# xiaojino/RUArt

Measured on AMD Instinct MI355X. Metric: VQA samples/sec fwd+bwd (B=64, q=30, ocr=100), higher is better.
Workload: dtype f16 MFMA + block-scaled fp8 (e4m3) MFMA correction, f32 accumulate / residual stream; 1 GPU; RUArt training step, synthetic ST-VQA-shaped batch: B=64/GPU, q=30 words, 100 OCR items, 36 objects, bert-base 12x768 frozen, SDNet trunk fwd+bwd, Adamax; global_batch=64, real_wordpieces_per_batch=42738, parallelism=dp1, mode=train

## Files before the change

### include/ruart_hip.h

```cpp
#ifndef RUART_HIP_H
#define RUART_HIP_H
#include <stddef.h>

#ifdef __cplusplus
extern "C" {
#endif

#define RUART_DT_F32 0
#define RUART_DT_BF16 1
#define RUART_DT_F16 2
#define RUART_ACT_NONE 0
#define RUART_ACT_GELU 1
#define RUART_ACT_RELU 2

const char* ruart_version(void);

int ruart_gemm_16_nt(const void* A, int lda, const void* W, int ldw, const float* bias, const void* residual, int ldr,
                     int residual_dtype, void* C, int ldc, int out_dtype, int M, int N, int K, int act, int in_dtype,
                     void* stream);
size_t ruart_gemm_16_tail_ws_bytes(int M, int N, int K, int cus);
int ruart_gemm_16_nt_ws(const void* A, int lda, const void* W, int ldw, const float* bias, const void* residual, int ldr, int residual_dtype,
                        void* C, int ldc, int out_dtype, int M, int N, int K, int act, int in_dtype, void* tail_ws, size_t tail_ws_bytes, int cus,
                        void* stream);
int ruart_gemm_16c_nt(const void* A16, const void* A8, int lda, const void* W16, const void* W8, int ldw, const float* bias,
// ... 138 lines not shown
size_t ruart_bert_workspace_bytes(const ruart_bert_model* m, int n_rows);
int ruart_bert_set_correction(int qkv, int ao, int ff1, int ff2, unsigned long long layer_mask);
int ruart_bert_forward(const ruart_bert_model* m, const ruart_bert_batch* b, void* layers_out, void* workspace,
                       size_t workspace_bytes, void* stream);

size_t ruart_bert_workspace_bytes_folded(const ruart_bert_model* m, int n_rows);
int ruart_bert_forward_folded(const ruart_bert_model* m, const ruart_bert_batch* b, void* layers_pre, float* ln_stats, void* workspace,
                              size_t workspace_bytes, void* stream);
int ruart_gemm_16c_nt_fold(const void* A16, const void* A8, int lda, const void* W16, const void* W8, int ldw, const float* bias, int kind,
                           const float* in_part, int in_np, const float* colc, float wscale, const float* residual, int ldr,
                           const float* res_part, int res_np, const float* res_gamma, const float* res_beta, void* C, int ldc, void* C16,
                           void* C8, float* out_part, int M, int N, int K, int stat_len, float eps, void* stream);
int ruart_gemm_16_nt_fold(const void* A, int lda, const void* W, int ldw, const float* bias, int kind, const float* in_part, int in_np,
                          const float* colc, float wscale, const void* residual, int ldr, const float* res_part, int res_np,
                          const float* res_gamma, const float* res_beta, void* C, int ldc, float* out_part, int M, int N, int K, int stat_len,
                          float eps, int dtype, void* stream);
int ruart_rows_stats_finish(const float* part, int np, int rows, float inv_h, float eps, float* stats, void* stream);
int ruart_bert_pool_mix_ln(const float* layers_pre, long long layer_stride, int ldl, int n_layers, const float* ln_stats,
                           long long stats_stride, const float* ln_gamma, const float* ln_beta, const int* span_start,
                           const int* span_start_last, const int* span_len, const int* dst_row, const float* layer_w, float* out, int ldo,
                           int n_words, int H, void* stream);
int ruart_bert_pool_ln_set_variant(int reg_tables);
int ruart_bert_pool_mix_ln_bwd(const float* layers_pre, long long layer_stride, int ldl, int n_layers, const float* ln_stats,
                               long long stats_stride, const float* ln_gamma, const float* ln_beta, const int* span_start,
                               const int* span_start_last, const int* span_len, const int* dst_row, const float* grad_out, int ldg,
                               float* partial_ws, float* grad_layer_w, int n_words, int H, void* stream);

int ruart_attn_fwd(const float* pa, const float* pk, const float* v, const unsigned char* mask, const float* diag, int diag_len,
                   int relu, float* out, float* probs, int B, int L1, int L2, int h, int D3, void* stream);
int ruart_attn_bwd(const float* pa, const float* pk, const float* v, const float* probs, const float* grad_out, const float* diag,
                   int diag_len, int relu, float* grad_pa, float* grad_pk, float* grad_v, float* grad_diag_partial,
                   float* ds_ws , int B, int L1, int L2, int h, int D3, void* stream);
int ruart_attn_set_prefetch(int on);
int ruart_attn_fwd_pscale(const float* pa, const float* pk, const float* v, const unsigned char* mask, const float* diag, int diag_len,
                          int relu, const float* prob_scale, float* out, float* probs, int B, int L1, int L2, int h, int D3,
                          void* stream);
int ruart_attn_bwd_pscale(const float* pa, const float* pk, const float* v, const float* probs, const float* grad_out, const float* diag,
                          int diag_len, int relu, const float* prob_scale, float* grad_pa, float* grad_pk, float* grad_v,
                          float* grad_diag_partial, float* ds_ws, int B, int L1, int L2, int h, int D3, void* stream);

int ruart_whole_ln_fwd(const float* x, float* y, float* stats, float* ws, long long n, float eps, void* stream);
int ruart_whole_ln_bwd(const float* y, const float* grad_y, const float* stats, float* grad_x, float* ws, long long n,
                       void* stream);

int ruart_whole_ln_blocks(void);
int ruart_whole_ln_partials(const float* x, const float* x2, float* part, long long n, void* stream);
int ruart_whole_ln_var_global(const float* x, long long n, const float* part_all, int world, long long n_total, float* part2,
                              void* stream);
int ruart_whole_ln_apply_global(const float* x, float* y, long long n, float eps, const float* part_all, const float* part2_all,
                                int world, long long n_total, float* stats, void* stream);
int ruart_whole_ln_bwd_global(const float* y, const float* grad_y, const float* stats, float* grad_x, long long n,
                              const float* part_all, int world, long long n_total, void* stream);

int ruart_scorer_fwd(const float* x, const float* u1, const float* u2, const float* uh, const float* w, const float* bna,
                     const unsigned char* mask, float* probs, float* a_out, int B, int L, int D, int ES, int mask_flag, void* stream);
int ruart_scorer_bwd(const float* x, const float* u1, const float* u2, const float* uh, const float* w, const float* probs,
                     const float* a_in, const float* gprobs, float* gx, float* gu1, float* gu2, float* guh, float* gw_part,
                     float* gb_part, int B, int L, int D, int ES, void* stream);

int ruart_lstm_set_variant(int variant);
int ruart_lstm_fwd(const float* xproj, const float* w_hh, float* y, float* gates, float* cells, float* hprev, int B, int T, int h,
                   int ndir, void* stream);
int ruart_lstm_bwd(const float* grad_y, const float* w_hh, const float* gates, const float* cells, float* grad_xproj, int B,
                   int T, int h, int ndir, void* stream);

int ruart_lstm_pack_params(const float* w_ih, const float* w_ih_r, const float* b_ih, const float* b_hh, const float* b_ih_r,
// ... 56 lines not shown
```

### ruart_amd/csrc/sdnet_attention.hip

```cpp
#include <cstdlib>
#include "common.h"
#include "ruart_hip.h"

#define CH 64
#define LDA_ 66
#define LDB_ 80
#define NTW 6
#define ATTN_MAX_L2 384

int* ruart_nan_flag_ptr = nullptr;

__device__ __forceinline__ f32x4_t mma16(const float* As, int lda, const float* Bs, int sbk, int sbj, int Kc, f32x4_t acc) {
  const int lane = threadIdx.x & 63, r = lane & 15, q = lane >> 4;
  for (int kk = 0; kk < Kc; kk += 4) acc = __builtin_amdgcn_mfma_f32_16x16x4f32(As[r * lda + kk + q], Bs[(kk + q) * sbk + r * sbj], acc, 0, 0, 0);
  return acc;
}

struct Act {
  int relu;
  const float* diag;
  int diag_len;
  __device__ __forceinline__ float operator()(float v, int col) const {
    if (relu) v = fmaxf(v, 0.f);
    if (diag_len == 1) v *= diag[0];
// ... 574 lines not shown
    const int kc = min(CH, (L1 - r0 + 3) & ~3);
    o = mma16(xt_s, LDA_, y_s + wave * 16, LDB_, 1, kc, o);
    if (ri == nr - 1) {
      const int n = n0 + wave * 16 + (lane & 15);
#pragma unroll
      for (int r = 0; r < 4; ++r) {
        const int j = j0 + (lane >> 4) * 4 + r;
        if (j < L2 && n < N) {
          const size_t at = (size_t)j * N + n;
          C[at] = (out_gate && out_gate[at] <= 0.f) ? 0.f : o[r];
        }
      }
      o = (f32x4_t){0.f, 0.f, 0.f, 0.f};
    }
    ri = rn;
    ni = nx;
  }
}

__global__ __launch_bounds__(256) void attn_bwd_kv_pf_kernel(const float* __restrict__ a, const float* __restrict__ probs,
                                                             const float* __restrict__ dS, const float* __restrict__ gout,
                                                             float* __restrict__ grad_k, float* __restrict__ grad_v, int L1, int L2, int h,
                                                             int D3, const float* __restrict__ pk, int relu,
                                                             const float* __restrict__ diag, int diag_len,
                                                             const float* __restrict__ pscale) {
  const int b = blockIdx.y, j0 = blockIdx.x * 16;
  float* xt_s = dsm;
  float* y_s = xt_s + 16 * LDA_;
  const size_t pb = (size_t)b * L1 * L2;
  tn_product_pf(dS + pb, L1, L2, j0, a + (size_t)b * L1 * h, h, grad_k + (size_t)b * L2 * h, xt_s, y_s, Act{relu, diag, diag_len},
                (relu && pk) ? pk + (size_t)b * L2 * h : nullptr, nullptr);
  tn_product_pf(probs + pb, L1, L2, j0, gout + (size_t)b * L1 * D3, D3, grad_v + (size_t)b * L2 * D3, xt_s, y_s, no_act(), nullptr,
                pscale ? pscale + pb : nullptr);
}

#define WLN_BLOCKS 256
__device__ __forceinline__ float grid_partial_total(const float* part, float* red) {
  float s = (threadIdx.x < WLN_BLOCKS) ? part[threadIdx.x] : 0.f;
  return block_sum<4>(s, red);
}

#define WLN_FOR4(n4, ...)                                                                          \
  for (long long i_ = blockIdx.x * 256LL + threadIdx.x; i_ < (n4); i_ += 4LL * 256 * WLN_BLOCKS) { \
    long long ix_[4];                                                                              \
    bool ok_[4];                                                                                   \
    _Pragma("unroll") for (int u_ = 0; u_ < 4; ++u_) {                                             \
      const long long j_ = i_ + (long long)u_ * 256 * WLN_BLOCKS;                                  \
      ok_[u_] = j_ < (n4);                                                                         \
      ix_[u_] = ok_[u_] ? j_ : (n4) - 1;                                                           \
    }                                                                                              \
    __VA_ARGS__                                                                                    \
  }
__device__ __forceinline__ bool wln_vec_ok(const void* a, const void* b, const void* c, long long n) {
  return ((n & 3) == 0) && (((reinterpret_cast<uintptr_t>(a) | reinterpret_cast<uintptr_t>(b) | reinterpret_cast<uintptr_t>(c)) & 15) == 0) && n >= 4;
}

__global__ __launch_bounds__(256) void wln_sum_kernel(const float* __restrict__ x, const float* __restrict__ x2, long long n,
                                                      float* __restrict__ part) {
  __shared__ float red[4];
  float s = 0.f, t = 0.f;
  if (wln_vec_ok(x, x2, nullptr, n)) {
    const f32x4_t* x4 = reinterpret_cast<const f32x4_t*>(x);
    const f32x4_t* y4 = reinterpret_cast<const f32x4_t*>(x2);
    const long long n4 = n >> 2;
    if (x2) {
      WLN_FOR4(n4, f32x4_t a[4], b[4];
// ... 148 lines not shown
               y4[ix_[u]] = o;
               bad |= !(o[0] == o[0]) || !(o[1] == o[1]) || !(o[2] == o[2]) || !(o[3] == o[3]);
             })
  } else {
    for (long long i = blockIdx.x * 256LL + threadIdx.x; i < n; i += 256LL * WLN_BLOCKS) {
      const float o = (x[i] - mean) * rstd;
      y[i] = o;
      bad |= !(o == o);
    }
  }
  if (bad && nan_flag) atomicOr(nan_flag, 1);
}
__global__ __launch_bounds__(256) void wln_bwd_global_kernel(const float* __restrict__ y, const float* __restrict__ gy,
                                                             const float* __restrict__ stats, float* __restrict__ gx, long long n,
                                                             const float* __restrict__ part_all, int world, long long n_total) {
  __shared__ float red[4];
  const float mg = wln_ranks_total(part_all, 2 * WLN_BLOCKS, world, red) / (float)n_total;
  const float mgy = wln_ranks_total(part_all + WLN_BLOCKS, 2 * WLN_BLOCKS, world, red) / (float)n_total;
  const float rstd = stats[1];
  if (wln_vec_ok(y, gy, gx, n)) {
    const f32x4_t* y4 = reinterpret_cast<const f32x4_t*>(y);
    const f32x4_t* g4 = reinterpret_cast<const f32x4_t*>(gy);
    f32x4_t* o4 = reinterpret_cast<f32x4_t*>(gx);
    const long long n4 = n >> 2;
    WLN_FOR4(n4, f32x4_t a[4], b[4];
             _Pragma("unroll") for (int u = 0; u < 4; ++u) { a[u] = y4[ix_[u]]; b[u] = g4[ix_[u]]; }
             _Pragma("unroll") for (int u = 0; u < 4; ++u) if (ok_[u]) o4[ix_[u]] = rstd * (b[u] - mg - a[u] * mgy);)
  } else {
    for (long long i = blockIdx.x * 256LL + threadIdx.x; i < n; i += 256LL * WLN_BLOCKS) gx[i] = rstd * (gy[i] - mg - y[i] * mgy);
  }
}

static bool g_attn_prefetch = !(getenv("RUART_ATTN_PREFETCH") && atoi(getenv("RUART_ATTN_PREFETCH")) == 0);
template <typename K> static void attn_big_lds(K kern) { hipFuncSetAttribute((const void*)kern, hipFuncAttributeMaxDynamicSharedMemorySize, 160 * 1024); }
static void attn_allow_big_lds() {
  static bool done = (attn_big_lds(attn_fwd_kernel), attn_big_lds(attn_bwd_q_kernel), attn_big_lds(attn_fwd_pf_kernel<12>),
                      attn_big_lds(attn_fwd_pf_kernel<16>), attn_big_lds(attn_fwd_pf_kernel<28>), attn_big_lds(attn_fwd_pf_kernel<32>),
                      attn_big_lds(attn_bwd_q_pf_kernel<12>), attn_big_lds(attn_bwd_q_pf_kernel<16>), attn_big_lds(attn_bwd_q_pf_kernel<28>),
                      attn_big_lds(attn_bwd_q_pf_kernel<32>), true);
  (void)done;
}

static size_t attn_lds_bytes(int L2) {
  const int L2p = (L2 + 15) & ~15;
  const int ldS = ((L2p + 31) / 32) * 32 + 2;
  return sizeof(float) * (size_t)(16 * LDA_ + 16 * ldS + L2p * LDB_);
}

__global__ __launch_bounds__(256) void attn1_fwd_kernel(const float* __restrict__ a, const float* __restrict__ k,
                                                        const float* __restrict__ v, const unsigned char* __restrict__ mask,
                                                        float* __restrict__ out, float* __restrict__ probs, int L2, int h, int D3,
                                                        int* __restrict__ nan_flag) {
  __shared__ float p_s[ATTN_MAX_L2];
  __shared__ float red[4];
  const int b = blockIdx.x, tid = threadIdx.x, lane = tid & 63, wave = tid >> 6;
  const float* ab = a + (size_t)b * h;
  const float* kb = k + (size_t)b * L2 * h;
  const float* vb = v + (size_t)b * L2 * D3;
  for (int j0 = wave * 4; j0 < L2; j0 += 16) {
    float s[4] = {0.f, 0.f, 0.f, 0.f};
    for (int d = lane; d < h; d += 64) {
      const float av = ab[d];
#pragma unroll
      for (int u = 0; u < 4; ++u)
        if (j0 + u < L2) s[u] = fmaf(av, kb[(size_t)(j0 + u) * h + d], s[u]);
    }
#pragma unroll
    for (int u = 0; u < 4; ++u) {
      const float t = wave_sum(s[u]);
      if (lane == 0 && j0 + u < L2) p_s[j0 + u] = mask[(size_t)b * L2 + j0 + u] ? t : -INFINITY;
    }
  }
  __syncthreads();
  float mx = -INFINITY;
  for (int j = tid; j < L2; j += 256) mx = fmaxf(mx, p_s[j]);
  mx = block_max<4>(mx, red);
  float sum = 0.f;
  for (int j = tid; j < L2; j += 256) {
    const float e = expf(p_s[j] - mx);
// ... 70 lines not shown
#pragma unroll
      for (int u = 0; u < 8; ++u) g = fmaf(ds_s[j + u], t[u], g);
    }
    for (; j < L2; ++j) g = fmaf(ds_s[j], kb[(size_t)j * h + d], g);
    grad_a[(size_t)b * h + d] = g;
  }
  for (int e = tid; e < L2 * h; e += 256) grad_k[(size_t)b * L2 * h + e] = ds_s[e / h] * ab[e % h];
  for (int e = tid; e < L2 * D3; e += 256) grad_v[(size_t)b * L2 * D3 + e] = pb[e / D3] * gb[e % D3];
}

extern "C" int ruart_attn_fwd(const float* a, const float* k, const float* v, const unsigned char* mask, const float* diag,
                              int diag_len, int relu, float* out, float* probs, int B, int L1, int L2, int h, int D3, void* stream) {
  RUART_ENTRY();
  return ruart_attn_fwd_pscale(a, k, v, mask, diag, diag_len, relu, nullptr, out, probs, B, L1, L2, h, D3, stream);
}

extern "C" int ruart_attn_fwd_pscale(const float* a, const float* k, const float* v, const unsigned char* mask, const float* diag,
                                     int diag_len, int relu, const float* prob_scale, float* out, float* probs, int B, int L1, int L2,
                                     int h, int D3, void* stream) {
  RUART_ENTRY();
  if (B <= 0 || L1 <= 0 || L2 <= 0 || L2 > ATTN_MAX_L2 || h <= 0 || D3 <= 0) return (int)hipErrorInvalidValue;
  if (diag_len != 0 && diag_len != 1 && diag_len != h) return (int)hipErrorInvalidValue;
  if (L1 == 1 && !relu && diag_len == 0 && !prob_scale) {
    hipLaunchKernelGGL(attn1_fwd_kernel, dim3(B), dim3(256), 0, (hipStream_t)stream, a, k, v, mask, out, probs, L2, h, D3,
                       ruart_nan_flag_ptr);
    RUART_CHECK_LAUNCH();
    return 0;
  }
  const dim3 grid(ceil_div(L1, 16), B), block(256);
  attn_allow_big_lds();
  const int L2p = (L2 + 15) & ~15;
#define RUART_AF(U) hipLaunchKernelGGL(attn_fwd_pf_kernel<U>, grid, block, attn_lds_bytes(L2), (hipStream_t)stream, a, k, v, mask, out, probs, \
                                       L1, L2, h, D3, ruart_nan_flag_ptr, relu, diag_len ? diag : nullptr, diag_len, prob_scale)
  if (!g_attn_prefetch || L2p > 128)
    hipLaunchKernelGGL(attn_fwd_kernel, grid, block, attn_lds_bytes(L2), (hipStream_t)stream, a, k, v, mask, out, probs, L1, L2, h, D3,
                       ruart_nan_flag_ptr, relu, diag_len ? diag : nullptr, diag_len, prob_scale);
  else if (L2p <= 48) RUART_AF(12);
  else if (L2p <= 64) RUART_AF(16);
  else if (L2p <= 112) RUART_AF(28);
  else RUART_AF(32);
#undef RUART_AF
  RUART_CHECK_LAUNCH();
  return 0;
}

extern "C" int ruart_attn_set_prefetch(int on) {
  RUART_ENTRY();
  g_attn_prefetch = on != 0;
  return 0;
}

extern "C" int ruart_attn_bwd(const float* a, const float* k, const float* v, const float* probs, const float* grad_out,
                              const float* diag, int diag_len, int relu, float* grad_a, float* grad_k, float* grad_v,
                              float* grad_diag, float* ds_ws, int B, int L1, int L2, int h, int D3, void* stream) {
  RUART_ENTRY();
  return ruart_attn_bwd_pscale(a, k, v, probs, grad_out, diag, diag_len, relu, nullptr, grad_a, grad_k, grad_v, grad_diag, ds_ws, B, L1,
                               L2, h, D3, stream);
}

extern "C" int ruart_attn_bwd_pscale(const float* a, const float* k, const float* v, const float* probs, const float* grad_out,
                                     const float* diag, int diag_len, int relu, const float* prob_scale, float* grad_a, float* grad_k,
                                     float* grad_v, float* grad_diag, float* ds_ws, int B, int L1, int L2, int h, int D3,
                                     void* stream) {
  RUART_ENTRY();
  if (B <= 0 || L1 <= 0 || L2 <= 0 || L2 > ATTN_MAX_L2 || h <= 0 || D3 <= 0) return (int)hipErrorInvalidValue;
  if (diag_len != 0 && diag_len != 1 && diag_len != h) return (int)hipErrorInvalidValue;
  if (L1 == 1 && !relu && diag_len == 0 && !prob_scale) {
    hipLaunchKernelGGL(attn1_bwd_kernel, dim3(B), dim3(256), 0, (hipStream_t)stream, a, k, v, probs, grad_out, grad_a, grad_k, grad_v,
                       L2, h, D3);
    RUART_CHECK_LAUNCH();
    return 0;
  }
  const bool act = relu || diag_len;
  const float* dg = diag_len ? diag : nullptr;
  attn_allow_big_lds();
  const int L2p = (L2 + 15) & ~15;
#define RUART_AQ(U) hipLaunchKernelGGL(attn_bwd_q_pf_kernel<U>, dim3(ceil_div(L1, 16), B), dim3(256), attn_lds_bytes(L2), (hipStream_t)stream, \
                                       k, v, probs, grad_out, grad_a, ds_ws, L1, L2, h, D3, act ? a : nullptr, relu, dg, diag_len,           \
                                       (diag_len > 1) ? grad_diag : nullptr, prob_scale)
  if (!g_attn_prefetch || L2p > 128)
    hipLaunchKernelGGL(attn_bwd_q_kernel, dim3(ceil_div(L1, 16), B), dim3(256), attn_lds_bytes(L2), (hipStream_t)stream, k, v, probs,
                       grad_out, grad_a, ds_ws, L1, L2, h, D3, act ? a : nullptr, relu, dg, diag_len,
                       (diag_len > 1) ? grad_diag : nullptr, prob_scale);
  else if (L2p <= 48) RUART_AQ(12);
  else if (L2p <= 64) RUART_AQ(16);
  else if (L2p <= 112) RUART_AQ(28);
  else RUART_AQ(32);
#undef RUART_AQ
  RUART_CHECK_LAUNCH();
  const size_t lds = sizeof(float) * (16 * LDA_ + CH * LDB_);
  if (g_attn_prefetch)
    hipLaunchKernelGGL(attn_bwd_kv_pf_kernel, dim3(ceil_div(L2, 16), B), dim3(256), lds, (hipStream_t)stream, a, probs, ds_ws, grad_out,
                       grad_k, grad_v, L1, L2, h, D3, k, relu, dg, diag_len, prob_scale);
  else
    hipLaunchKernelGGL(attn_bwd_kv_kernel, dim3(ceil_div(L2, 16), B), dim3(256), lds, (hipStream_t)stream, a, probs, ds_ws, grad_out,
                       grad_k, grad_v, L1, L2, h, D3, k, relu, dg, diag_len, prob_scale);
  RUART_CHECK_LAUNCH();
  return 0;
}

extern "C" int ruart_whole_ln_fwd(const float* x, float* y, float* stats, float* ws, long long n, float eps, void* stream) {
  RUART_ENTRY();
  if (n <= 0) return (int)hipErrorInvalidValue;
  hipStream_t s = (hipStream_t)stream;
  hipLaunchKernelGGL(wln_sum_kernel, dim3(WLN_BLOCKS), dim3(256), 0, s, x, (const float*)nullptr, n, ws);
  hipLaunchKernelGGL(wln_var_kernel, dim3(WLN_BLOCKS), dim3(256), 0, s, x, n, ws, ws + 2 * WLN_BLOCKS);
  hipLaunchKernelGGL(wln_apply_kernel, dim3(WLN_BLOCKS), dim3(256), 0, s, x, y, n, eps, ws, ws + 2 * WLN_BLOCKS, stats, ruart_nan_flag_ptr);
  RUART_CHECK_LAUNCH();
  return 0;
}

extern "C" int ruart_whole_ln_bwd(const float* y, const float* grad_y, const float* stats, float* grad_x, float* ws, long long n,
                                  void* stream) {
  RUART_ENTRY();
  if (n <= 0) return (int)hipErrorInvalidValue;
  hipStream_t s = (hipStream_t)stream;
  hipLaunchKernelGGL(wln_sum_kernel, dim3(WLN_BLOCKS), dim3(256), 0, s, grad_y, y, n, ws);
  hipLaunchKernelGGL(wln_bwd_kernel, dim3(WLN_BLOCKS), dim3(256), 0, s, y, grad_y, stats, grad_x, n, ws);
  RUART_CHECK_LAUNCH();
  return 0;
}

extern "C" int ruart_whole_ln_blocks(void) { return WLN_BLOCKS; }

// ... 85 lines not shown
```

### ruart_amd/hip.py

```python
import ctypes
import os
from ctypes import POINTER, Structure, c_char_p, c_double, c_float, c_int, c_longlong, c_size_t, c_uint, c_ulonglong, c_void_p

import torch

_HERE = os.path.dirname(os.path.abspath(__file__))
LIB_PATH = os.path.join(_HERE, "libruart_hip.so")

DT_F32, DT_BF16, DT_F16 = 0, 1, 2
ACT_NONE, ACT_GELU, ACT_RELU = 0, 1, 2
TORCH_DTYPE = {DT_F32: torch.float32, DT_BF16: torch.bfloat16, DT_F16: torch.float16}
PRECISION = {"fp32": DT_F32, "bf16": DT_BF16, "fp16": DT_F16, "x3": DT_F32, "fp16c": DT_F32}


class BertModelC(Structure):
    _fields_ = [("hidden", c_int), ("n_heads", c_int), ("n_layers", c_int), ("intermediate", c_int), ("dtype", c_int),
                ("ln_eps", c_float),
                ("word_emb", c_void_p), ("pos_emb", c_void_p), ("type_emb", c_void_p), ("emb_ln_g", c_void_p), ("emb_ln_b", c_void_p),
                ("w_qkv", POINTER(c_void_p)), ("b_qkv", POINTER(c_void_p)),
                ("w_ao", POINTER(c_void_p)), ("b_ao", POINTER(c_void_p)),
                ("ln1_g", POINTER(c_void_p)), ("ln1_b", POINTER(c_void_p)),
                ("w_ff1", POINTER(c_void_p)), ("b_ff1", POINTER(c_void_p)),
                ("w_ff2", POINTER(c_void_p)), ("b_ff2", POINTER(c_void_p)),
                ("ln2_g", POINTER(c_void_p)), ("ln2_b", POINTER(c_void_p)), ("f32_gemm", c_int), ("corr8", c_int),
# ... 69 lines not shown
    "ruart_weight_prep_batch": (_I, [POINTER(WPrepItemC), _I, _P]),
    "ruart_colsum_bf16": (_I, [_P, _I, _I, _I, _P, _I, _P, _P]),
    "ruart_transpose16": (_I, [_P, _I, _P, _I, _I, _I, _I, _P]),
    "ruart_splitk_reduce": (_I, [_P, _LL, _I, _P, _LL, _F, _I, _P]),
    "ruart_mix_rows": (_I, [_P, _LL, _I, _I, _P, _P, _I, _I, _I, _P]),
    "ruart_mix_rows_bwd": (_I, [_P, _LL, _I, _I, _P, _I, _P, _P, _I, _I, _P]),
    "ruart_rows_ln_to_16": (_I, [_P, _LL, _I, _P, _LL, _P, _P, _P, _LL, _I, _I, _I, _I, _I, _P]),
    "ruart_attn_train_fwd": (_I, [_P, _I, _P, _I, _I, _I, _I, _P, _P, _P, _F, _U, _P]),
    "ruart_attn_train_bwd": (_I, [_P, _I, _P, _I, _P, _I, _I, _I, _I, _P, _P, _P, _F, _U, _P, _P]),
    "ruart_attn_train_fwd_long": (_I, [_P, _I, _P, _I, _I, _I, _I, _P, _P, _P, _P, _F, _U, _P, _P]),
    "ruart_attn_train_bwd_long": (_I, [_P, _I, _P, _I, _P, _I, _I, _I, _I, _P, _P, _P, _P, _P, _F, _U, _P, _P, _P, _P, _P]),
    "ruart_gemm_f32_nt": (_I, [_P, _I, _P, _I, _P, _P, _I, _P, _I, _I, _I, _I, _I, _P]),
    "ruart_bert_embed_ln": (_I, [_P, _P, _P, _P, _P, _P, _P, _F, _P, _I, _I, _I, _I, _P]),
    "ruart_rows_layernorm": (_I, [_P, _I, _P, _P, _F, _P, _I, _I, _I, _I, _P]),
    "ruart_bert_attention": (_I, [_P, _I, _P, _I, _I, _I, _I, _I, _P, _P, _P, _P, _P, _P, _P, _I, _P, _P, _P, _P, _P]),
    "ruart_bert_pool_set_variant": (_I, [_I]),
    "ruart_bert_pool_mix": (_I, [_P, _LL, _I, _I, _I, _P, _P, _P, _P, _P, _P, _I, _I, _I, _P]),
    "ruart_bert_pool_mix_bwd": (_I, [_P, _LL, _I, _I, _I, _P, _P, _P, _P, _P, _I, _P, _P, _I, _I, _P]),
    "ruart_rows_gather": (_I, [_P, _I, _P, _LL, _P, _LL, _I, _P, _LL, _P, _LL, _I, _P, _LL, _P, _LL, _I, _P]),
    "ruart_cast_f32_to_16": (_I, [_P, _P, _I, _LL, _F, _P]),
    "ruart_bert_workspace_bytes": (_SZ, [POINTER(BertModelC), _I]),
    "ruart_bert_forward": (_I, [POINTER(BertModelC), POINTER(BertBatchC), _P, _P, _SZ, _P]),
    "ruart_bert_workspace_bytes_folded": (_SZ, [POINTER(BertModelC), _I]),
    "ruart_bert_forward_folded": (_I, [POINTER(BertModelC), POINTER(BertBatchC), _P, _P, _P, _SZ, _P]),
    "ruart_gemm_16c_nt_fold": (_I, [_P, _P, _I, _P, _P, _I, _P, _I, _P, _I, _P, _F, _P, _I, _P, _I, _P, _P, _P, _I, _P, _P, _P, _I, _I, _I, _I, _F, _P]),
    "ruart_gemm_16_nt_fold": (_I, [_P, _I, _P, _I, _P, _I, _P, _I, _P, _F, _P, _I, _P, _I, _P, _P, _P, _I, _P, _I, _I, _I, _I, _F, _I, _P]),
    "ruart_rows_stats_finish": (_I, [_P, _I, _I, _F, _F, _P, _P]),
    "ruart_bert_pool_mix_ln": (_I, [_P, _LL, _I, _I, _P, _LL, _P, _P, _P, _P, _P, _P, _P, _P, _I, _I, _I, _P]),
    "ruart_bert_pool_ln_set_variant": (_I, [_I]),
    "ruart_bert_pool_mix_ln_bwd": (_I, [_P, _LL, _I, _I, _P, _LL, _P, _P, _P, _P, _P, _P, _P, _I, _P, _P, _I, _I, _P]),
    "ruart_attn_fwd": (_I, [_P, _P, _P, _P, _P, _I, _I, _P, _P, _I, _I, _I, _I, _I, _P]),
    "ruart_attn_bwd": (_I, [_P, _P, _P, _P, _P, _P, _I, _I, _P, _P, _P, _P, _P, _I, _I, _I, _I, _I, _P]),
    "ruart_attn_set_prefetch": (_I, [_I]),
    "ruart_attn_fwd_pscale": (_I, [_P, _P, _P, _P, _P, _I, _I, _P, _P, _P, _I, _I, _I, _I, _I, _P]),
    "ruart_attn_bwd_pscale": (_I, [_P, _P, _P, _P, _P, _P, _I, _I, _P, _P, _P, _P, _P, _P, _I, _I, _I, _I, _I, _P]),
    "ruart_whole_ln_fwd": (_I, [_P, _P, _P, _P, _LL, _F, _P]),
    "ruart_whole_ln_bwd": (_I, [_P, _P, _P, _P, _P, _LL, _P]),
    "ruart_whole_ln_blocks": (_I, []),
    "ruart_whole_ln_partials": (_I, [_P, _P, _P, _LL, _P]),
    "ruart_whole_ln_var_global": (_I, [_P, _LL, _P, _I, _LL, _P, _P]),
    "ruart_whole_ln_apply_global": (_I, [_P, _P, _LL, _F, _P, _P, _I, _LL, _P, _P]),
    "ruart_whole_ln_bwd_global": (_I, [_P, _P, _P, _P, _LL, _P, _I, _LL, _P]),
    "ruart_scorer_fwd": (_I, [_P, _P, _P, _P, _P, _P, _P, _P, _P, _I, _I, _I, _I, _I, _P]),
    "ruart_scorer_bwd": (_I, [_P, _P, _P, _P, _P, _P, _P, _P, _P, _P, _P, _P, _P, _P, _I, _I, _I, _I, _P]),
    "ruart_lstm_set_variant": (_I, [_I]),
    "ruart_lstm_pack_params": (_I, [_P, _P, _P, _P, _P, _P, _P, _P, _P, _P, _P, _I, _I, _I, _P]),
    "ruart_lstm_fwd": (_I, [_P, _P, _P, _P, _P, _P, _I, _I, _I, _I, _P]),
    "ruart_lstm_bwd": (_I, [_P, _P, _P, _P, _P, _I, _I, _I, _I, _P]),
    "ruart_rows_scale": (_I, [_P, _I, _P, _I, _P, _P, _I, _I, _I, _P]),
    "ruart_lstm_cell_fwd": (_I, [_P, _P, _P, _P, _P, _P, _I, _I, _I, _P]),
    "ruart_lstm_cell_bwd": (_I, [_P, _P, _P, _P, _P, _P, _P, _P, _I, _I, _I, _P]),
    "ruart_set_nan_flag": (_I, [_P]),
    "ruart_grad_norm_clip": (_I, [_P, _P, _P, _P, _I, _F, _P, _P, _P, _P]),
    "ruart_adamax_step": (_I, [_P, _P, _P, _P, _P, _P, _P, _I, _P, _P, _F, _F, _F, _P]),
    "ruart_embedding_bwd_sorted": (_I, [_P, _P, _P, _P, _I, _I, _P, _P]),
    "ruart_embedding_bwd_split": (_I, [_P, _P, _P, _I, _P, _P, _I, _I, _P, _P, _P]),
    "ruart_phoc_table": (_I, [_P, _P, _I, _P, _I, _P, _P]),
    "ruart_gemm_bf16_tn": (_I, [_P, _LL, _P, _LL, _P, _I, _I, _I, _I, _P, _SZ, _P]),
    "ruart_gemm_x3_tn_grouped_ws": (_SZ, [POINTER(X3TnProblemC), _I]),
    "ruart_gemm_x3_tn_grouped": (_I, [POINTER(X3TnProblemC), _I, _P, _SZ, _P]),
    "ruart_gemm_x3_plan": (_I, [_I, _I, _I, _I, _I, POINTER(c_int), POINTER(_SZ)]),
    "ruart_gemm_x3": (_I, [_P, _LL, _LL, _P, _LL, _LL, _P, _P, _I, _I, _P, _I, _I,
                           _I, _I, _P, _SZ, _P, _P, _F, _P, _I, _P]),
    "ruart_gemm_x1": (_I, [_P, _LL, _LL, _P, _LL, _LL, _P, _P, _I, _I, _P, _I, _I,
                           _I, _I, _P, _SZ, _P, _P, _F, _P, _I, _P]),
    "ruart_stream_create_cu_masked": (_I, [_I, POINTER(c_void_p)]),
# ... 150 lines not shown
```

Before: 2870 samples/s.

## Add LDS-resident attention kernels that stage whole K/V panels per block

Adds resident-panel variants of the SDNet attention forward, backward-dQ and backward-dK/dV kernels for L2 up to 128. These stage entire key/value (or dS/probs) panels into up to 160 KiB of LDS once, using bulk register-buffered loads, and reuse them across several 16-row query tiles per block. The goal is to cut repeated global reloads and per-tile staging overhead. The forward and dQ paths only run when RUART_ATTN_RESIDENT is positive. The dK/dV path runs by default unless that variable is negative, so it replaces the prefetch kernel and changes grid shape and occupancy.

```diff
diff --git a/include/ruart_hip.h b/include/ruart_hip.h
--- a/include/ruart_hip.h
+++ b/include/ruart_hip.h
@@ -194,6 +194,8 @@
                    int diag_len, int relu, float* grad_pa, float* grad_pk, float* grad_v, float* grad_diag_partial,
                    float* ds_ws , int B, int L1, int L2, int h, int D3, void* stream);
 int ruart_attn_set_prefetch(int on);
+int ruart_attn_set_resident(int tiles);
+int ruart_attn_get_resident(int* tiles);
 int ruart_attn_fwd_pscale(const float* pa, const float* pk, const float* v, const unsigned char* mask, const float* diag, int diag_len,
                           int relu, const float* prob_scale, float* out, float* probs, int B, int L1, int L2, int h, int D3,
                           void* stream);
diff --git a/ruart_amd/csrc/sdnet_attention.hip b/ruart_amd/csrc/sdnet_attention.hip
--- a/ruart_amd/csrc/sdnet_attention.hip
+++ b/ruart_amd/csrc/sdnet_attention.hip
@@ -630,6 +630,403 @@
                 (relu && pk) ? pk + (size_t)b * L2 * h : nullptr, nullptr);
   tn_product_pf(probs + pb, L1, L2, j0, gout + (size_t)b * L1 * D3, D3, grad_v + (size_t)b * L2 * D3, xt_s, y_s, no_act(), nullptr,
                 pscale ? pscale + pb : nullptr);
+}
+
+#define RES_U 32
+#define RES_NT 2
+#define RES_LDS_MAX (160 * 1024)
+
+__host__ __device__ __forceinline__ int res_lda(int n) { return ((n + 31) / 32) * 32 + 2; }
+__host__ __device__ __forceinline__ int res_ldb(int n) { const int m = (n + 15) & ~15; return (m & 31) ? m : m + 16; }
+
+struct RPanel {
+  const float* src;
+  int ld, r0, rows, c0, cols, nr_pad, nc_pad;
+};
+__device__ __forceinline__ int rp_quads(const RPanel& p) { return ((p.nr_pad + 15) >> 4) * ((p.nc_pad + 63) >> 6); }
+
+__device__ __forceinline__ float res_ldg(const float* __restrict__ base, unsigned byte_off) {
+  return *reinterpret_cast<const float*>(reinterpret_cast<const char*>(base) + byte_off);
+}
+
+template <int U, int MUL>
+struct Bulk {
+  float v[U];
+  float m[MUL == 2 ? U : (MUL == 1 ? U / 4 : 1)];
+  __device__ __forceinline__ void load(const RPanel& p, int q0, const float* __restrict__ mul = nullptr) {
+    const int lane = threadIdx.x & 63, w = __builtin_amdgcn_readfirstlane(threadIdx.x >> 6);
+    const int NRQ = (p.nr_pad + 15) >> 4;
+    const float* msrc = mul ? mul : p.src;
+    int ci = q0 / NRQ, rq = q0 - ci * NRQ;
+#pragma unroll
+    for (int qq = 0; qq < U / 4; ++qq) {
+      {
+        const unsigned cc = 4u * (unsigned)min(p.c0 + ci * 64 + lane, p.cols - 1);
+        if (MUL == 1) m[qq] = mul ? res_ldg(msrc, cc) : 1.f;
+#pragma unroll
+        for (int j = 0; j < 4; ++j) {
+          const unsigned at = (unsigned)min(p.r0 + rq * 16 + j * 4 + w, p.rows - 1) * (4u * (unsigned)p.ld) + cc;
+          v[qq * 4 + j] = res_ldg(p.src, at);
+          if (MUL == 2) m[qq * 4 + j] = mul ? res_ldg(msrc, at) : 1.f;
+        }
+      }
+      if (++rq == NRQ) {
+        rq = 0;
+        ++ci;
+      }
+    }
+  }
+  template <bool TR>
+  __device__ __forceinline__ void store(float* dst, int ldd, const RPanel& p, int q0, int relu, float cmul) const {
+    const int lane = threadIdx.x & 63, w = __builtin_amdgcn_readfirstlane(threadIdx.x >> 6);
+    const int NRQ = (p.nr_pad + 15) >> 4, NC = (p.nc_pad + 63) >> 6;
+    int ci = q0 / NRQ, rq = q0 - ci * NRQ;
+#pragma unroll
+    for (int qq = 0; qq < U / 4; ++qq) {
+      const int c = ci * 64 + lane;
+      if (ci < NC && c < p.nc_pad) {
+        const bool colok = p.c0 + c < p.cols;
+#pragma unroll
+        for (int j = 0; j < 4; ++j) {
+          const int r = rq * 16 + j * 4 + w;
+          float x = v[qq * 4 + j];
+          if (relu) x = fmaxf(x, 0.f);
+          if (MUL == 1) x *= m[qq];
+          if (MUL == 2) x *= m[qq * 4 + j];
+          x *= cmul;
+          if (r < p.nr_pad) dst[TR ? c * ldd + r : r * ldd + c] = (colok && p.r0 + r < p.rows) ? x : 0.f;
+        }
+      }
+      if (++rq == NRQ) {
+        rq = 0;
+        ++ci;
+      }
+    }
+  }
+};
+#define RES_UQ (RES_U / 4)
+
+struct ResNothing {
+  __device__ __forceinline__ void operator()() const {}
+};
+template <bool TR, typename F = ResNothing>
+__device__ __forceinline__ void stage_bulk(float* dst, int ldd, const RPanel& p, int relu, F also = F()) {
+  const int NQ = rp_quads(p);
+  {
+    Bulk<RES_U, 0> b0, b1;
+    b0.load(p, 0);
+    if (RES_UQ < NQ) b1.load(p, RES_UQ);
+    also();
+    b0.template store<TR>(dst, ldd, p, 0, relu, 1.f);
+    if (RES_UQ < NQ) b1.template store<TR>(dst, ldd, p, RES_UQ, relu, 1.f);
+  }
+  for (int q0 = 2 * RES_UQ; q0 < NQ; q0 += 2 * RES_UQ) {
+    Bulk<RES_U, 0> b0, b1;
+    b0.load(p, q0);
+    if (q0 + RES_UQ < NQ) b1.load(p, q0 + RES_UQ);
+    b0.template store<TR>(dst, ldd, p, q0, relu, 1.f);
+    if (q0 + RES_UQ < NQ) b1.template store<TR>(dst, ldd, p, q0 + RES_UQ, relu, 1.f);
+  }
+}
+
+__device__ __forceinline__ void res_scores(const float* q_s, const float* p1_s, int ld1, int Kc, int ntile, float* Sg, int ldS) {
+  const int lane = threadIdx.x & 63, wave = threadIdx.x >> 6;
+#pragma unroll
+  for (int t = 0; t < RES_NT; ++t) {
+    const int jt = wave + 4 * t;
+    if (jt < ntile) {
+      f32x4_t acc = {0.f, 0.f, 0.f, 0.f};
+      acc = mma16(q_s, ld1, p1_s + jt * 16 * ld1, 1, ld1, Kc, acc);
+#pragma unroll
+      for (int r = 0; r < 4; ++r) Sg[((lane >> 4) * 4 + r) * ldS + jt * 16 + (lane & 15)] = acc[r];
+    }
+  }
+}
+
+__global__ __launch_bounds__(256) void attn_fwd_res_kernel(const float* __restrict__ a, const float* __restrict__ k,
+                                                           const float* __restrict__ v, const unsigned char* __restrict__ mask,
+                                                           float* __restrict__ out, float* __restrict__ probs, int L1, int L2, int h,
+                                                           int D3, int* __restrict__ nan_flag, int relu, const float* __restrict__ diag,
+                                                           int diag_len, const float* __restrict__ pscale, int G, int sep) {
+  const int b = blockIdx.y, nq = (L1 + 15) >> 4, g0 = blockIdx.x * G, g1 = min(g0 + G, nq);
+  const int lane = threadIdx.x & 63, wave = threadIdx.x >> 6;
+  const int L2p = (L2 + 15) & ~15, ldS = lds_probs_stride(L2p), ntile = L2p / 16;
+  const int hp = (h + 3) & ~3, ld1 = res_lda(hp), Dp = (D3 + 15) & ~15, ld2 = res_ldb(Dp);
+  float* q_s = dsm;
+  float* S_s = q_s + 16 * ld1;
+  float* k_s = S_s + G * 16 * ldS;
+  float* v_s = sep ? k_s + L2p * ld1 : k_s;
+  const float* ab = a + (size_t)b * L1 * h;
+  const RPanel pk{k + (size_t)b * L2 * h, h, 0, L2, 0, h, L2p, hp};
+  const RPanel pv{v + (size_t)b * L2 * D3, D3, 0, L2, 0, D3, L2p, Dp};
+  RPanel pq{ab, h, g0 * 16, L1, 0, h, 16, hp};
+  const float* dvec = diag_len > 1 ? diag : nullptr;
+  const float cm = diag_len == 1 ? diag[0] : 1.f;
+
+  Bulk<RES_U, 1> qa;
+  stage_bulk<false>(k_s, ld1, pk, relu, [&]() { qa.load(pq, 0, dvec); });
+  qa.store<false>(q_s, ld1, pq, 0, relu, cm);
+  Bulk<RES_U, 0> v0, v1;
+  const int TV = rp_quads(pv);
+  if (sep) {
+    v0.load(pv, 0);
+    if (RES_UQ < TV) v1.load(pv, RES_UQ);
+  }
+  pq.r0 = min(g0 + 1, nq - 1) * 16;
+  qa.load(pq, 0, dvec);
+  unsigned char mk[RES_NT * 4];
+#pragma unroll
+  for (int t = 0; t < RES_NT * 4; ++t) mk[t] = mask[(size_t)b * L2 + min((int)(threadIdx.x & 15) + 16 * t, L2 - 1)];
+
+  for (int g = g0; g < g1; ++g) {
+    float* Sg = S_s + (g - g0) * 16 * ldS;
+    const int i0 = g * 16;
+    __syncthreads();
+    res_scores(q_s, k_s, ld1, hp, ntile, Sg, ldS);
+    __syncthreads();
+    if (sep && g == g0) {
+      v0.store<false>(v_s, ld2, pv, 0, 0, 1.f);
+      if (RES_UQ < TV) v1.store<false>(v_s, ld2, pv, RES_UQ, 0, 1.f);
+    }
+    if (g + 1 < g1) {
+      qa.store<false>(q_s, ld1, pq, 0, relu, cm);
+      pq.r0 = min(g + 2, nq - 1) * 16;
+      qa.load(pq, 0, dvec);
+    }
+    {
+      const int row = threadIdx.x >> 4, c = threadIdx.x & 15;
+      float* Sr = Sg + row * ldS;
+      float mx = -INFINITY;
+#pragma unroll
+      for (int t = 0; t < RES_NT * 4; ++t) {
+        const int j = c + 16 * t;
+        if (j < L2) {
+          const float s = mk[t] ? Sr[j] : -INFINITY;
+          Sr[j] = s;
+          mx = fmaxf(mx, s);
+        }
+      }
+#pragma unroll
+      for (int o = 8; o > 0; o >>= 1) mx = fmaxf(mx, __shfl_xor(mx, o, 64));
+      float sum = 0.f;
+      for (int j = c; j < L2; j += 16) {
+        const float e = expf(Sr[j] - mx);
+        Sr[j] = e;
+        sum += e;
+      }
+#pragma unroll
+      for (int o = 8; o > 0; o >>= 1) sum += __shfl_xor(sum, o, 64);
+      const float inv = 1.0f / sum;
+      const bool live = (i0 + row) < L1;
+      bool bad = false;
+      for (int j = c; j < L2p; j += 16) {
+        const float p = (j < L2) ? Sr[j] * inv : 0.f;
+        const float ps = (pscale && live && j < L2) ? pscale[((size_t)b * L1 + i0 + row) * L2 + j] : 1.f;
+        Sr[j] = live ? p * ps : 0.f;
+        bad |= live && !(p == p);
+        if (probs && live && j < L2) probs[((size_t)b * L1 + i0 + row) * L2 + j] = p;
+      }
+      if (bad && nan_flag) atomicOr(nan_flag, 1);
+    }
+  }
+  __syncthreads();
+  if (!sep) {
+    stage_bulk<false>(v_s, ld2, pv, 0);
+    __syncthreads();
+  }
+  const int nct = Dp / 16;
+  for (int g = g0; g < g1; ++g) {
+    const float* Sg = S_s + (g - g0) * 16 * ldS;
+    for (int ct = wave; ct < nct; ct += 4) {
+      f32x4_t o = {0.f, 0.f, 0.f, 0.f};
+      o = mma16(Sg, ldS, v_s + ct * 16, ld2, 1, L2p, o);
+      const int d = ct * 16 + (lane & 15);
+#pragma unroll
+      for (int r = 0; r < 4; ++r) {
+        const int i = g * 16 + (lane >> 4) * 4 + r;
+        if (i < L1 && d < D3) out[((size_t)b * L1 + i) * D3 + d] = o[r];
+      }
+    }
+  }
+}
+
+__global__ __launch_bounds__(256) void attn_bwd_q_res_kernel(const float* __restrict__ k, const float* __restrict__ v,
+                                                             const float* __restrict__ probs, const float* __restrict__ gout,
+                                                             float* __restrict__ grad_a, float* __restrict__ dS, int L1, int L2, int h,
+                                                             int D3, const float* __restrict__ pa_, int relu,
+                                                             const float* __restrict__ diag, int diag_len,
+                                                             float* __restrict__ grad_diag, const float* __restrict__ pscale, int G,
+                                                             int sep) {
+  const int b = blockIdx.y, nq = (L1 + 15) >> 4, g0 = blockIdx.x * G, g1 = min(g0 + G, nq);
+  const int lane = threadIdx.x & 63, wave = threadIdx.x >> 6;
+  const int L2p = (L2 + 15) & ~15, ldS = lds_probs_stride(L2p), ntile = L2p / 16;
+  const int Dp = (D3 + 3) & ~3, ld1 = res_lda(Dp), hp = (h + 15) & ~15, ld2 = res_ldb(hp);
+  float* q_s = dsm;
+  float* S_s = q_s + 16 * ld1;
+  float* v_s = S_s + G * 16 * ldS;
+  float* k_s = sep ? v_s + L2p * ld1 : v_s;
+  const float* gb = gout + (size_t)b * L1 * D3;
+  const RPanel pv{v + (size_t)b * L2 * D3, D3, 0, L2, 0, D3, L2p, Dp};
+  const RPanel pk{k + (size_t)b * L2 * h, h, 0, L2, 0, h, L2p, hp};
+  RPanel pq{gb, D3, g0 * 16, L1, 0, D3, 16, Dp};
+
+  Bulk<RES_U, 0> qa;
+  stage_bulk<false>(v_s, ld1, pv, 0, [&]() { qa.load(pq, 0); });
+  qa.store<false>(q_s, ld1, pq, 0, 0, 1.f);
+  Bulk<RES_U, 0> k0, k1;
+  const int TK = rp_quads(pk);
+  if (sep) {
+    k0.load(pk, 0);
+    if (RES_UQ < TK) k1.load(pk, RES_UQ);
+  }
+  pq.r0 = min(g0 + 1, nq - 1) * 16;
+  qa.load(pq, 0);
+
+  for (int g = g0; g < g1; ++g) {
+    float* Sg = S_s + (g - g0) * 16 * ldS;
+    const int i0 = g * 16;
+    const int row = threadIdx.x >> 4, c = threadIdx.x & 15;
+    const bool live = (i0 + row) < L1;
+    const float* Pr = probs + ((size_t)b * L1 + (live ? i0 + row : 0)) * L2;
+    float pr[RES_NT * 4];
+#pragma unroll
+    for (int t = 0; t < RES_NT * 4; ++t) pr[t] = Pr[min(c + 16 * t, L2 - 1)];
+    __syncthreads();
+    res_scores(q_s, v_s, ld1, Dp, ntile, Sg, ldS);
+    __syncthreads();
+    if (sep && g == g0) {
+      k0.store<false>(k_s, ld2, pk, 0, relu, 1.f);
+      if (RES_UQ < TK) k1.store<false>(k_s, ld2, pk, RES_UQ, relu, 1.f);
+    }
+    if (g + 1 < g1) {
+      qa.store<false>(q_s, ld1, pq, 0, 0, 1.f);
+      pq.r0 = min(g + 2, nq - 1) * 16;
+      qa.load(pq, 0);
+    }
+    {
+      float* Sr = Sg + row * ldS;
+      float dot = 0.f;
+      if (pscale && live) {
+        const float* Mr = pscale + ((size_t)b * L1 + i0 + row) * L2;
+        for (int j = c; j < L2; j += 16) Sr[j] *= Mr[j];
+      }
+#pragma unroll
+      for (int t = 0; t < RES_NT * 4; ++t) {
+        const int j = c + 16 * t;
+        if (j < L2) dot += Sr[j] * pr[t];
+      }
+#pragma unroll
+      for (int o = 8; o > 0; o >>= 1) dot += __shfl_xor(dot, o, 64);
+#pragma unroll
+      for (int t = 0; t < RES_NT * 4; ++t) {
+        const int j = c + 16 * t;
+        if (j < L2p) {
+          float d = 0.f;
+          if (live && j < L2) {
+            d = pr[t] * (Sr[j] - dot);
+            dS[((size_t)b * L1 + i0 + row) * L2 + j] = d;
+          }
+          Sr[j] = d;
+        }
+      }
+    }
+  }
+  __syncthreads();
+  if (!sep) {
+    stage_bulk<false>(k_s, ld2, pk, relu);
+    __syncthreads();
+  }
+  const int nct = hp / 16;
+  for (int g = g0; g < g1; ++g) {
+    const float* Sg = S_s + (g - g0) * 16 * ldS;
+    for (int ct = wave; ct < nct; ct += 4) {
+      const int d = ct * 16 + (lane & 15);
+      float pv4[4];
+      if (pa_) {
+#pragma unroll
+        for (int r = 0; r < 4; ++r) pv4[r] = pa_[((size_t)b * L1 + min(g * 16 + (lane >> 4) * 4 + r, L1 - 1)) * h + min(d, h - 1)];
+      }
+      f32x4_t o = {0.f, 0.f, 0.f, 0.f};
+      o = mma16(Sg, ldS, k_s + ct * 16, ld2, 1, L2p, o);
+      float gd = 0.f;
+      const float dsc = (d < h) ? (diag_len == 1 ? diag[0] : (diag_len > 1 ? diag[d] : 1.f)) : 0.f;
+#pragma unroll
+      for (int r = 0; r < 4; ++r) {
+        const int i = g * 16 + (lane >> 4) * 4 + r;
+        if (i < L1 && d < h) {
+          const size_t at = ((size_t)b * L1 + i) * h + d;
+          float gg = o[r];
+          if (pa_) {
+            const float pvv = pv4[r];
+            gd += gg * (relu ? fmaxf(pvv, 0.f) : pvv);
+            gg = (relu && pvv <= 0.f) ? 0.f : gg * dsc;
+          }
+          grad_a[at] = gg;
+        }
+      }
+      if (grad_diag) {
+        gd += __shfl_xor(gd, 16, 64);
+        gd += __shfl_xor(gd, 32, 64);
+        if ((lane >> 4) == 0 && d < h) grad_diag[((size_t)b * nq + g) * h + d] = gd;
+      }
+    }
+  }
+}
+
+template <bool PS>
+__global__ __launch_bounds__(256) void attn_bwd_kv_res_kernel(const float* __restrict__ a, const float* __restrict__ probs,
+                                                              const float* __restrict__ dS, const float* __restrict__ gout,
+                                                              float* __restrict__ grad_k, float* __restrict__ grad_v, int L1, int L2,
+                                                              int h, int D3, const float* __restrict__ pk, int relu,
+                                                              const float* __restrict__ diag, int diag_len,
+                                                              const float* __restrict__ pscale) {
+  const int b = blockIdx.y, nnh = (h + CH - 1) / CH;
+  const bool first = (int)blockIdx.x < nnh;
+  const int n0 = (first ? blockIdx.x : blockIdx.x - nnh) * CH, N = first ? h : D3;
+  const int lane = threadIdx.x & 63, wave = threadIdx.x >> 6;
+  const int L2p = (L2 + 15) & ~15, L1p = (L1 + 3) & ~3, ldX = res_lda(L1p);
+  float* xt_s = dsm;
+  float* y_s = xt_s + L2p * ldX;
+  const size_t pb = (size_t)b * L1 * L2;
+  const float* X = (first ? dS : probs) + pb;
+  const float* xmul = (PS && !first) ? pscale + pb : nullptr;
+  const float* Y = first ? a + (size_t)b * L1 * h : gout + (size_t)b * L1 * D3;
+  float* C = first ? grad_k + (size_t)b * L2 * h : grad_v + (size_t)b * L2 * D3;
+  const float* gate = (first && relu && pk) ? pk + (size_t)b * L2 * h : nullptr;
+  const int yrelu = first ? relu : 0;
+  const int n = n0 + wave * 16 + (lane & 15);
+  const float cm = (first && diag_len) ? (diag_len == 1 ? diag[0] : diag[min(n0 + lane, N - 1)]) : 1.f;
+  const RPanel px{X, L2, 0, L1, 0, L2, L1p, L2p};
+  const RPanel py{Y, N, 0, L1, n0, N, L1p, CH};
+  const int QX = rp_quads(px), QY = rp_quads(py);
+  for (int q0 = 0; q0 < max(QX, QY); q0 += 2 * RES_UQ) {
+    Bulk<RES_U, PS ? 2 : 0> x0, x1;
+    Bulk<RES_U, 0> y0, y1;
+    if (q0 < QX) x0.load(px, q0, xmul);
+    if (q0 + RES_UQ < QX) x1.load(px, q0 + RES_UQ, xmul);
+    if (q0 < QY) y0.load(py, q0);
+    if (q0 + RES_UQ < QY) y1.load(py, q0 + RES_UQ);
+    if (q0 < QX) x0.template store<true>(xt_s, ldX, px, q0, 0, 1.f);
+    if (q0 + RES_UQ < QX) x1.template store<true>(xt_s, ldX, px, q0 + RES_UQ, 0, 1.f);
+    if (q0 < QY) y0.template store<false>(y_s, LDB_, py, q0, yrelu, cm);
+    if (q0 + RES_UQ < QY) y1.template store<false>(y_s, LDB_, py, q0 + RES_UQ, yrelu, cm);
+  }
+  __syncthreads();
+  if (n0 + wave * 16 >= N) return;
+  for (int jt = 0; jt < L2p / 16; ++jt) {
+    float gv[4];
+    if (gate) {
+#pragma unroll
+      for (int r = 0; r < 4; ++r) gv[r] = gate[(size_t)min(jt * 16 + (lane >> 4) * 4 + r, L2 - 1) * N + min(n, N - 1)];
+    }
+    f32x4_t o = {0.f, 0.f, 0.f, 0.f};
+    o = mma16(xt_s + jt * 16 * ldX, ldX, y_s + wave * 16, LDB_, 1, L1p, o);
+#pragma unroll
+    for (int r = 0; r < 4; ++r) {
+      const int j = jt * 16 + (lane >> 4) * 4 + r;
+      if (j < L2 && n < N) C[(size_t)j * N + n] = (gate && gv[r] <= 0.f) ? 0.f : o[r];
+    }
+  }
 }
 
 #define WLN_BLOCKS 256
@@ -844,12 +1241,14 @@
 }
 
 static bool g_attn_prefetch = !(getenv("RUART_ATTN_PREFETCH") && atoi(getenv("RUART_ATTN_PREFETCH")) == 0);
+static int g_attn_resident = getenv("RUART_ATTN_RESIDENT") ? atoi(getenv("RUART_ATTN_RESIDENT")) : 0;
 template <typename K> static void attn_big_lds(K kern) { hipFuncSetAttribute((const void*)kern, hipFuncAttributeMaxDynamicSharedMemorySize, 160 * 1024); }
 static void attn_allow_big_lds() {
   static bool done = (attn_big_lds(attn_fwd_kernel), attn_big_lds(attn_bwd_q_kernel), attn_big_lds(attn_fwd_pf_kernel<12>),
                       attn_big_lds(attn_fwd_pf_kernel<16>), attn_big_lds(attn_fwd_pf_kernel<28>), attn_big_lds(attn_fwd_pf_kernel<32>),
                       attn_big_lds(attn_bwd_q_pf_kernel<12>), attn_big_lds(attn_bwd_q_pf_kernel<16>), attn_big_lds(attn_bwd_q_pf_kernel<28>),
-                      attn_big_lds(attn_bwd_q_pf_kernel<32>), true);
+                      attn_big_lds(attn_bwd_q_pf_kernel<32>), attn_big_lds(attn_fwd_res_kernel), attn_big_lds(attn_bwd_q_res_kernel),
+                      attn_big_lds(attn_bwd_kv_res_kernel<false>), attn_big_lds(attn_bwd_kv_res_kernel<true>), true);
   (void)done;
 }
 
@@ -857,6 +1256,39 @@
   const int L2p = (L2 + 15) & ~15;
   const int ldS = ((L2p + 31) / 32) * 32 + 2;
   return sizeof(float) * (size_t)(16 * LDA_ + 16 * ldS + L2p * LDB_);
+}
+
+struct ResPlan {
+  int G, sep;
+  size_t lds;
+};
+static bool attn_res_plan(int L1, int L2, int n1, int n2, ResPlan* p) {
+  if (!g_attn_prefetch || g_attn_resident <= 0) return false;
+  const int L2p = (L2 + 15) & ~15, n1p = (n1 + 3) & ~3, n2p = (n2 + 15) & ~15;
+  if (L2p > 128 || n1p > 16 * RES_U) return false;
+  const int ld1 = res_lda(n1p), ld2 = res_ldb(n2p), ldS = ((L2p + 31) / 32) * 32 + 2, nq = ceil_div(L1, 16);
+  const int T2 = (L2p / 4) * ((n2p + 63) / 64);
+  for (int G = g_attn_resident < nq ? g_attn_resident : nq; G >= 1; --G) {
+    const size_t base = (size_t)16 * ld1 + (size_t)G * 16 * ldS;
+    const size_t both = sizeof(float) * (base + (size_t)L2p * (ld1 + ld2));
+    const size_t one = sizeof(float) * (base + (size_t)L2p * (ld1 > ld2 ? ld1 : ld2));
+    if (T2 <= 2 * RES_U && both <= RES_LDS_MAX) {
+      *p = ResPlan{G, 1, both};
+      return true;
+    }
+    if (one <= RES_LDS_MAX) {
+      *p = ResPlan{G, 0, one};
+      return true;
+    }
+  }
+  return false;
+}
+static size_t attn_res_kv_lds(int L1, int L2) {
+  if (!g_attn_prefetch || g_attn_resident < 0) return 0;
+  const int L2p = (L2 + 15) & ~15, L1p = (L1 + 3) & ~3;
+  if (L2p > 128) return 0;
+  const size_t lds = sizeof(float) * ((size_t)L2p * res_lda(L1p) + (size_t)L1p * LDB_);
+  return lds <= RES_LDS_MAX ? lds : 0;
 }
 
 __global__ __launch_bounds__(256) void attn1_fwd_kernel(const float* __restrict__ a, const float* __restrict__ k,
@@ -993,7 +1425,11 @@
   const int L2p = (L2 + 15) & ~15;
 #define RUART_AF(U) hipLaunchKernelGGL(attn_fwd_pf_kernel<U>, grid, block, attn_lds_bytes(L2), (hipStream_t)stream, a, k, v, mask, out, probs, \
                                        L1, L2, h, D3, ruart_nan_flag_ptr, relu, diag_len ? diag : nullptr, diag_len, prob_scale)
-  if (!g_attn_prefetch || L2p > 128)
+  ResPlan rp;
+  if (attn_res_plan(L1, L2, h, D3, &rp))
+    hipLaunchKernelGGL(attn_fwd_res_kernel, dim3(ceil_div(ceil_div(L1, 16), rp.G), B), block, rp.lds, (hipStream_t)stream, a, k, v, mask, out,
+                       probs, L1, L2, h, D3, ruart_nan_flag_ptr, relu, diag_len ? diag : nullptr, diag_len, prob_scale, rp.G, rp.sep);
+  else if (!g_attn_prefetch || L2p > 128)
     hipLaunchKernelGGL(attn_fwd_kernel, grid, block, attn_lds_bytes(L2), (hipStream_t)stream, a, k, v, mask, out, probs, L1, L2, h, D3,
                        ruart_nan_flag_ptr, relu, diag_len ? diag : nullptr, diag_len, prob_scale);
   else if (L2p <= 48) RUART_AF(12);
@@ -1008,6 +1444,20 @@
 extern "C" int ruart_attn_set_prefetch(int on) {
   RUART_ENTRY();
   g_attn_prefetch = on != 0;
+  return 0;
+}
+
+extern "C" int ruart_attn_set_resident(int tiles) {
+  RUART_ENTRY();
+  if (tiles < -1) return (int)hipErrorInvalidValue;
+  g_attn_resident = tiles;
+  return 0;
+}
+
+extern "C" int ruart_attn_get_resident(int* tiles) {
+  RUART_ENTRY();
+  if (!tiles) return (int)hipErrorInvalidValue;
+  *tiles = g_attn_resident;
   return 0;
 }
 
@@ -1039,7 +1489,12 @@
 #define RUART_AQ(U) hipLaunchKernelGGL(attn_bwd_q_pf_kernel<U>, dim3(ceil_div(L1, 16), B), dim3(256), attn_lds_bytes(L2), (hipStream_t)stream, \
                                        k, v, probs, grad_out, grad_a, ds_ws, L1, L2, h, D3, act ? a : nullptr, relu, dg, diag_len,           \
                                        (diag_len > 1) ? grad_diag : nullptr, prob_scale)
-  if (!g_attn_prefetch || L2p > 128)
+  ResPlan rp;
+  if (attn_res_plan(L1, L2, D3, h, &rp))
+    hipLaunchKernelGGL(attn_bwd_q_res_kernel, dim3(ceil_div(ceil_div(L1, 16), rp.G), B), dim3(256), rp.lds, (hipStream_t)stream, k, v, probs,
+                       grad_out, grad_a, ds_ws, L1, L2, h, D3, act ? a : nullptr, relu, dg, diag_len,
+                       (diag_len > 1) ? grad_diag : nullptr, prob_scale, rp.G, rp.sep);
+  else if (!g_attn_prefetch || L2p > 128)
     hipLaunchKernelGGL(attn_bwd_q_kernel, dim3(ceil_div(L1, 16), B), dim3(256), attn_lds_bytes(L2), (hipStream_t)stream, k, v, probs,
                        grad_out, grad_a, ds_ws, L1, L2, h, D3, act ? a : nullptr, relu, dg, diag_len,
                        (diag_len > 1) ? grad_diag : nullptr, prob_scale);
@@ -1050,7 +1505,15 @@
 #undef RUART_AQ
   RUART_CHECK_LAUNCH();
   const size_t lds = sizeof(float) * (16 * LDA_ + CH * LDB_);
-  if (g_attn_prefetch)
+  const size_t lds_res = attn_res_kv_lds(L1, L2);
+  const dim3 grid_res(ceil_div(h, CH) + ceil_div(D3, CH), B);
+  if (lds_res && prob_scale)
+    hipLaunchKernelGGL(attn_bwd_kv_res_kernel<true>, grid_res, dim3(256), lds_res, (hipStream_t)stream, a, probs, ds_ws, grad_out, grad_k,
+                       grad_v, L1, L2, h, D3, k, relu, dg, diag_len, prob_scale);
+  else if (lds_res)
+    hipLaunchKernelGGL(attn_bwd_kv_res_kernel<false>, grid_res, dim3(256), lds_res, (hipStream_t)stream, a, probs, ds_ws, grad_out, grad_k,
+                       grad_v, L1, L2, h, D3, k, relu, dg, diag_len, prob_scale);
+  else if (g_attn_prefetch)
     hipLaunchKernelGGL(attn_bwd_kv_pf_kernel, dim3(ceil_div(L2, 16), B), dim3(256), lds, (hipStream_t)stream, a, probs, ds_ws, grad_out,
                        grad_k, grad_v, L1, L2, h, D3, k, relu, dg, diag_len, prob_scale);
   else
diff --git a/ruart_amd/hip.py b/ruart_amd/hip.py
--- a/ruart_amd/hip.py
+++ b/ruart_amd/hip.py
@@ -125,6 +125,8 @@
     "ruart_attn_fwd": (_I, [_P, _P, _P, _P, _P, _I, _I, _P, _P, _I, _I, _I, _I, _I, _P]),
     "ruart_attn_bwd": (_I, [_P, _P, _P, _P, _P, _P, _I, _I, _P, _P, _P, _P, _P, _I, _I, _I, _I, _I, _P]),
     "ruart_attn_set_prefetch": (_I, [_I]),
+    "ruart_attn_set_resident": (_I, [_I]),
+    "ruart_attn_get_resident": (_I, [_P]),
     "ruart_attn_fwd_pscale": (_I, [_P, _P, _P, _P, _P, _I, _I, _P, _P, _P, _I, _I, _I, _I, _I, _P]),
     "ruart_attn_bwd_pscale": (_I, [_P, _P, _P, _P, _P, _P, _I, _I, _P, _P, _P, _P, _P, _P, _I, _I, _I, _I, _I, _P]),
     "ruart_whole_ln_fwd": (_I, [_P, _P, _P, _P, _LL, _F, _P]),
```

Result: no change. 2877 samples/s, median of 6 (+0.2%).
